# Rayman96/Paddle_ray

Hardware: AMD Instinct MI355X
Metric: tokens/sec GPT-3-1.3B Fleet sharding-3 (higher is better)
Workload: dtype bf16; 1 GPU; model=GPT-3-1.3B, global_batch=16, seq_len=1024, parallelism=sharding3_dp1, micro_batch_per_gpu=16, optimizer=AdamW fp32-master, global-norm clip, zero3_active=False, zero3_params=n/a (world 1)

## Files before the change

paddle_ray_amd/ops/csrc/flash_attn.hip:

```cpp
#include "common.h"
#include "pra_api.h"
#include <stdlib.h>
#include <string.h>
#include <type_traits>
#include <algorithm>
#include <cmath>

namespace pra {
namespace fa {

__device__ __forceinline__ float fexp2(float x) { return __builtin_amdgcn_exp2f(x); }

__device__ __forceinline__ void wait_vmem_all() { __builtin_amdgcn_s_waitcnt(0x0F70); }

typedef float f32x16 __attribute__((ext_vector_type(16)));
typedef uint32_t u32x4 __attribute__((ext_vector_type(4)));
typedef uint32_t u32x2 __attribute__((ext_vector_type(2)));

template <typename T> struct V8;
template <> struct V8<bf16> { typedef __bf16 type __attribute__((ext_vector_type(8))); };
template <> struct V8<f16> { typedef _Float16 type __attribute__((ext_vector_type(8))); };

template <typename T>
__device__ __forceinline__ f32x16 mfma(typename V8<T>::type a, typename V8<T>::type b, f32x16 c);
template <>
__device__ __forceinline__ f32x16 mfma<bf16>(V8<bf16>::type a, V8<bf16>::type b, f32x16 c) {
  return __builtin_amdgcn_mfma_f32_32x32x16_bf16(a, b, c, 0, 0, 0);
}
template <>
__device__ __forceinline__ f32x16 mfma<f16>(V8<f16>::type a, V8<f16>::type b, f32x16 c) {
  return __builtin_amdgcn_mfma_f32_32x32x16_f16(a, b, c, 0, 0, 0);
}

template <typename T> __device__ __forceinline__ uint32_t pack2(float a, float b);
template <> __device__ __forceinline__ uint32_t pack2<bf16>(float a, float b) { return pack_bf2(a, b); }
template <> __device__ __forceinline__ uint32_t pack2<f16>(float a, float b) {
  _Float16 x = (_Float16)a, y = (_Float16)b;
  return (uint32_t)__builtin_bit_cast(uint16_t, x) | ((uint32_t)__builtin_bit_cast(uint16_t, y) << 16);
}
template <typename T> __device__ __forceinline__ float lo16(uint32_t w);
template <typename T> __device__ __forceinline__ float hi16(uint32_t w);
template <> __device__ __forceinline__ float lo16<bf16>(uint32_t w) { return __uint_as_float(w << 16); }
template <> __device__ __forceinline__ float hi16<bf16>(uint32_t w) { return __uint_as_float(w & 0xffff0000u); }
template <> __device__ __forceinline__ float lo16<f16>(uint32_t w) {
  return (float)__builtin_bit_cast(_Float16, (uint16_t)(w & 0xffff));
}
template <> __device__ __forceinline__ float hi16<f16>(uint32_t w) {
  return (float)__builtin_bit_cast(_Float16, (uint16_t)(w >> 16));
}

template <typename T>
__device__ __forceinline__ typename V8<T>::type as_v8(u32x4 u) {
  return __builtin_bit_cast(typename V8<T>::type, u);
}
template <typename T>
__device__ __forceinline__ typename V8<T>::type pack_frag(const f32x16& acc, int base) {
  u32x4 u;
  u[0] = pack2<T>(acc[base + 0], acc[base + 1]);
  u[1] = pack2<T>(acc[base + 2], acc[base + 3]);
  u[2] = pack2<T>(acc[base + 4], acc[base + 5]);
  u[3] = pack2<T>(acc[base + 6], acc[base + 7]);
  return as_v8<T>(u);
}

constexpr int kTile = 64;

struct FaExt {
  const int* cu_q;
  const int* cu_k;
  const void* mask;
  int64_t msb, msh, msq;
  int mask_f32;
  float mask_mul;
  uint32_t thr;
  float inv_keep;
  uint64_t seed, offset;
  uint32_t* dbits;
  int dbits_ld;
  int xf;
  const uint64_t* dseq;
  float* bsum;
  int bsum_nblk;
};

enum : int { XF_DROP = 1, XF_KMASK = 2, XF_FMASK = 4 };

__device__ __forceinline__ uint32_t fa_mix32(uint32_t x) {
  x ^= x >> 16; x *= 0x7feb352dU; x ^= x >> 15; x *= 0x846ca68bU; x ^= x >> 16;
  return x;
}
__device__ __forceinline__ uint32_t fa_key(const FaExt& e, int bh) {
  const uint64_t seed = e.dseq ? e.seed ^ (*e.dseq * 0x9E3779B97F4A7C15ull) : e.seed;
  return fa_mix32((uint32_t)seed ^ (uint32_t)(seed >> 32) * 0x27d4eb2fU ^
                  (uint32_t)e.offset * 0x165667b1U ^ (uint32_t)bh * 0xc2b2ae3dU);
}
__device__ __forceinline__ uint32_t fa_hash2(uint32_t key, int q, int kpair) {
  return fa_mix32(key ^ (uint32_t)q * 0x9e3779b1U ^ (uint32_t)kpair * 0x85ebca77U);
}
__device__ __forceinline__ float fa_keep(const FaExt& e, uint32_t u16) { return u16 >= e.thr ? e.inv_keep : 0.f; }
__device__ __forceinline__ float fa_drop(const FaExt& e, uint32_t key, int q, int kk) {
  const uint32_t hs = fa_hash2(key, q, kk >> 1);
  return fa_keep(e, (kk & 1) ? (hs >> 16) : (hs & 0xffffu));
}
template <typename T>
__device__ __forceinline__ float fa_mask(const FaExt& e, int b, int hh, int q, int kk) {
  const int64_t i = (int64_t)b * e.msb + (int64_t)hh * e.msh + (int64_t)q * e.msq + kk;
  float m;
  if (e.mask_f32) m = static_cast<const float*>(e.mask)[i];
  else m = Cvt<T>::to(static_cast<const T*>(e.mask)[i]);
  return m * e.mask_mul;
}

template <int D>
__device__ __forceinline__ int swz(int row, int ch) {
  return (row >> 3) * (8 * D) + (ch >> 2) * 256 + (row & 7) * 32 + 8 * ((ch & 3) ^ ((row >> 2) & 3));
}
// ... 302 lines not shown
          const uint32_t hs = fa_hash2(dkey, myq, kk >> 1);
          const bool keep = ((i & 1) ? (hs >> 16) : (hs & 0xffffu)) >= ext.thr;
          kbits[mt] |= keep ? (1u << acc_row(i, 0)) : 0u;
          p = keep ? p : 0.f;
        }
        s_acc[mt][i] = p;
      }
    if constexpr ((XF & XF_DROP) != 0) {
      if (ext.dbits) {
#pragma unroll
        for (int mt = 0; mt < 2; ++mt) {
          const uint32_t kb = kbits[mt] << (4 * h);
          const uint32_t w = kb | __shfl_xor(kb, 32, 64);
          if (h == 0 && myq < Sq && mt < nlive)
            ext.dbits[((int64_t)bh * SqM + myq) * ext.dbits_ld + (k0 >> 5) + mt] = w;
        }
      }
    }
    ps += __shfl_xor(ps, 32, 64);
    l_run += ps;
#pragma unroll
    for (int ks = 0; ks < 4; ++ks) {
      if (ks < 2 * nlive) {
        const typename V8<T>::type pf = pack_frag<T>(s_acc[ks >> 1], 8 * (ks & 1));
#pragma unroll
        for (int dt = 0; dt < ND; ++dt)
          acc_o[dt] = mfma<T>(ks < 2 ? vfr[ks & 1][dt] : frag_tr<T, D>(Vs, lo, dt, ks), pf, acc_o[dt]);
      }
    }
    }
    asm volatile("s_waitcnt vmcnt(0)" ::: "memory");
    __syncthreads();
  };
  int nfull = min(ntiles, Sk / kTile);
  if (CAUSAL) nfull = min(nfull, (q0 + off + 1) / kTile);
  if (nfull < 0) nfull = 0;
  auto run = [&](auto xf_c) __attribute__((always_inline)) {
    for (int kt = 0; kt < nfull; ++kt) tile(kt, std::false_type{}, xf_c);
    for (int kt = nfull; kt < ntiles; ++kt) tile(kt, std::true_type{}, xf_c);
  };
  if constexpr (!EXT) {
    run(std::integral_constant<int, 0>{});
  } else {
    switch (ext.xf) {
      case XF_DROP: run(std::integral_constant<int, XF_DROP>{}); break;
      case XF_KMASK: run(std::integral_constant<int, XF_KMASK>{}); break;
      case XF_KMASK | XF_DROP: run(std::integral_constant<int, XF_KMASK | XF_DROP>{}); break;
      case XF_FMASK: run(std::integral_constant<int, XF_FMASK>{}); break;
      case XF_FMASK | XF_DROP: run(std::integral_constant<int, XF_FMASK | XF_DROP>{}); break;
      default: run(std::integral_constant<int, 0>{}); break;
    }
  }

  if (myq < Sq) {
    float inv = l_run > 0.f ? 1.f / l_run : 0.f;
    if constexpr (EXT) {
      if (ext.xf & XF_DROP) inv *= ext.inv_keep;
    }
    T* orow = o + (qrow0 + myq) * ((int64_t)H * D) + (int64_t)hh * D;
#pragma unroll
    for (int dt = 0; dt < ND; ++dt)
#pragma unroll
      for (int g = 0; g < 4; ++g) {
        const int d = 32 * dt + 8 * g + 4 * h;
        uint2 w;
        w.x = pack2<T>(acc_o[dt][4 * g + 0] * inv, acc_o[dt][4 * g + 1] * inv);
        w.y = pack2<T>(acc_o[dt][4 * g + 2] * inv, acc_o[dt][4 * g + 3] * inv);
        *reinterpret_cast<uint2*>(orow + d) = w;
      }
    if (h == 0) {
      const float l2 = l_run > 0.f ? (m_run + log2f(l_run)) : INFINITY;
      lse[(int64_t)bh * SqM + myq] = l2 * 0.6931471805599453f;
    }
  }
}

template <typename T, int D, bool CAUSAL, int NW>
__global__ void __launch_bounds__(NW * 64, 2)
bwd_dq_kernel(const T* __restrict__ q, const T* __restrict__ k, const T* __restrict__ v, const T* __restrict__ dO,
              const T* __restrict__ o, const float* __restrict__ lse, float* __restrict__ delta, T* __restrict__ dq, int H, int Sq,
              int Sk, int64_t qsb, int64_t qss, int64_t qsh, int64_t ksb, int64_t kss, int64_t ksh, int64_t vsb,
              int64_t vss, int64_t vsh, int64_t dqsb, int64_t dqss, int64_t dqsh, float scale, float scale_log2) {
  extern __shared__ __attribute__((aligned(16))) char smem[];
  T* img0 = reinterpret_cast<T*>(smem);
  constexpr int NS = D / 16, ND = D / 32, BM = NW * 32;
  const float LOG2E = 1.4426950408889634f;

  const int nqb = gridDim.y;
  const int qb = CAUSAL ? (nqb - 1 - blockIdx.y) : blockIdx.y;
  const int bh = blockIdx.x, b = bh / H, hh = bh % H;
  const int wave = threadIdx.x >> 6, lane = threadIdx.x & 63, r = lane & 31, h = lane >> 5;
  const int q0 = qb * BM;
  const int myq = q0 + wave * 32 + r;
  const int off = Sk - Sq;
  const bool qvalid = myq < Sq;

  const T* qb_ = q + b * qsb + hh * qsh;
  const T* kb_ = k + b * ksb + hh * ksh;
  const T* vb_ = v + b * vsb + hh * vsh;
  const int64_t HD = (int64_t)H * D;
  const T* dob_ = dO + (int64_t)b * Sq * HD + (int64_t)hh * D;

  typename V8<T>::type qf[NS], df[NS];
  {
    const int qq = qvalid ? myq : 0;
#pragma unroll
    for (int s = 0; s < NS; ++s) {
      qf[s] = frag_global<T>(qb_ + (int64_t)qq * qss, 16 * s + 8 * h, qvalid);
      df[s] = frag_global<T>(dob_ + (int64_t)qq * HD, 16 * s + 8 * h, qvalid);
    }
  }
  const float lse2 = qvalid ? lse[(int64_t)bh * Sq + myq] * LOG2E : INFINITY;
  float dlt;
  if (o) {
    const T* ob_ = o + (int64_t)b * Sq * HD + (int64_t)hh * D;
    const int qq = qvalid ? myq : 0;
    float part = 0.f;
#pragma unroll
    for (int s = 0; s < NS; ++s) {
      const typename V8<T>::type of = frag_global<T>(ob_ + (int64_t)qq * HD, 16 * s + 8 * h, qvalid);
      const u32x4 uo = __builtin_bit_cast(u32x4, of), ud = __builtin_bit_cast(u32x4, df[s]);
#pragma unroll
      for (int j = 0; j < 4; ++j)
// ... 52 lines not shown
#pragma unroll
      for (int g = 0; g <= NG; ++g) {
        if (g < NG) {
#pragma unroll
          for (int j = 0; j < G; ++j) {
            const int f = g * G + j;
            fr[g & 1][j] = f < NS ? frag_rows<T, D>(Ks, lo, mt, f) : frag_rows<T, D>(Vs, lo, mt, f - NS);
          }
        }
        if (g > 0) {
#pragma unroll
          for (int j = 0; j < G; ++j) {
            const int f = (g - 1) * G + j;
            if (f < NS) s_acc[mt] = mfma<T>(fr[(g - 1) & 1][j], qf[f], s_acc[mt]);
            else dp_acc[mt] = mfma<T>(fr[(g - 1) & 1][j], df[f - NS], dp_acc[mt]);
          }
        }
        __builtin_amdgcn_sched_barrier(0);
      }
    }
#pragma unroll
    for (int mt = 0; mt < 2; ++mt)
#pragma unroll
      for (int i = 0; i < 16; ++i) {
        float p = fexp2(fmaf(s_acc[mt][i], scale_log2, -lse2));
        if constexpr (MASK) {
          const int key = k0 + 32 * mt + acc_row(i, h);
          if (mt >= nlive || key >= Sk || (CAUSAL && key > myq + off)) p = 0.f;
        }
        s_acc[mt][i] = p * (dp_acc[mt][i] - dlt);
      }
#pragma unroll
    for (int ks = 0; ks < 4; ++ks) {
      if (ks < 2 * nlive) {
        const typename V8<T>::type sf = pack_frag<T>(s_acc[ks >> 1], 8 * (ks & 1));
#pragma unroll
        for (int dt = 0; dt < ND; ++dt) acc_q[dt] = mfma<T>(frag_tr<T, D>(Ks, lo, dt, ks), sf, acc_q[dt]);
      }
    }
    }
    if (kt + 1 < ntiles) {
      T* nb = img0 + (2 * ((kt + 1) & 1)) * kTile * D;
      kr.store_swz(nb);
      vr.store_swz(nb + kTile * D);
    }
    __syncthreads();
  };
  int nfull = min(ntiles, Sk / kTile);
  if (CAUSAL) nfull = min(nfull, (q0 + off + 1) / kTile);
  if (nfull < 0) nfull = 0;
  for (int kt = 0; kt < nfull; ++kt) tile(kt, std::false_type{});
  for (int kt = nfull; kt < ntiles; ++kt) tile(kt, std::true_type{});

  if (qvalid) {
    T* row = dq + (int64_t)b * dqsb + (int64_t)myq * dqss + (int64_t)hh * dqsh;
#pragma unroll
    for (int dt = 0; dt < ND; ++dt)
#pragma unroll
      for (int g = 0; g < 4; ++g) {
        const int d = 32 * dt + 8 * g + 4 * h;
        uint2 w;
        w.x = pack2<T>(acc_q[dt][4 * g + 0] * scale, acc_q[dt][4 * g + 1] * scale);
        w.y = pack2<T>(acc_q[dt][4 * g + 2] * scale, acc_q[dt][4 * g + 3] * scale);
        *reinterpret_cast<uint2*>(row + d) = w;
      }
  }
}

template <typename T, int D, bool EXT, int NWV = 4>
__host__ __device__ constexpr int kKvOff() {
  return 4 * kTile * D * (int)sizeof(T) + 4 * kTile * 4 + NWV * 32 * 80 + (EXT ? 2 * 256 * 4 : 0);
}
template <typename T, int D, bool EXT, int NWV = 4>
__host__ __device__ constexpr int kDkdvLds() {
  return kKvOff<T, D, EXT, NWV>() + 4 * kTile * D * (int)sizeof(T);
}
__host__ __device__ constexpr int dkdv_waves(bool qs) { return qs ? 8 : 4; }

template <typename T, int D, bool CAUSAL, bool WDS, bool EXT = false, bool QS = false>
__global__ void __launch_bounds__(64 * dkdv_waves(QS), (D == 64 && !QS) ? 2 : 1)
bwd_dkdv_kernel(const T* __restrict__ q, const T* __restrict__ k, const T* __restrict__ v, const T* __restrict__ dO,
                const float* __restrict__ lse, const float* __restrict__ delta, T* __restrict__ dk,
                T* __restrict__ dv, int H, int SqM, int SkM, int64_t qsb, int64_t qss, int64_t qsh, int64_t ksb,
                int64_t kss, int64_t ksh, int64_t vsb, int64_t vss, int64_t vsh, int64_t dksb, int64_t dkss,
                int64_t dksh, int64_t dvsb, int64_t dvss, int64_t dvsh, float scale, float scale_log2,
                T* __restrict__ dsT, int Sqp, int64_t dsbh, FaExt ext = {}) {
  extern __shared__ __attribute__((aligned(16))) char smem[];
  T* img0 = reinterpret_cast<T*>(smem);
  float* Lsb = reinterpret_cast<float*>(img0 + 4 * kTile * D);
  float* Dlb = Lsb + 2 * kTile;
  constexpr int NS = D / 16, ND = D / 32;
  const float LOG2E = 1.4426950408889634f;

  constexpr int NWV = dkdv_waves(QS), NTH = 64 * NWV;
  const int kb = blockIdx.y;
  const int bh = blockIdx.x, b = bh / H, hh = bh % H;
  const int wave = threadIdx.x >> 6, lane = threadIdx.x & 63, r = lane & 31, h = lane >> 5;
  const int kw = QS ? (wave & 3) : wave, qh = QS ? (wave >> 2) : 0;
  const int kblk0 = kb * 128;
  const int mykey = kblk0 + kw * 32 + r;
  int Sq = SqM, Sk = SkM;
  int64_t qrow0 = (int64_t)b * SqM, krow0 = 0;
  if constexpr (EXT) {
    if (ext.cu_q) {
      qrow0 = ext.cu_q[b];
      krow0 = ext.cu_k[b];
      Sq = ext.cu_q[b + 1] - (int)qrow0;
      Sk = ext.cu_k[b + 1] - (int)krow0;
      if (kblk0 >= Sk) return;
    }
  }
  const int off = Sk - Sq;
  const bool kvalid = mykey < Sk;
  const bool vl = EXT && ext.cu_q;

  const T* qb_ = vl ? q + qrow0 * qss + hh * qsh : q + b * qsb + hh * qsh;
  const T* kb_ = vl ? k + krow0 * kss + hh * ksh : k + b * ksb + hh * ksh;
  const T* vb_ = vl ? v + krow0 * vss + hh * vsh : v + b * vsb + hh * vsh;
  const int64_t HD = (int64_t)H * D;
  const T* dob_ = dO + qrow0 * HD + (int64_t)hh * D;

  const T* kvimg = reinterpret_cast<const T*>(smem + kKvOff<T, D, EXT, NWV>());
  const T* Kw = kvimg + (kw >> 1) * kTile * D;
  const T* Vw = kvimg + (2 + (kw >> 1)) * kTile * D;
  f32x16 acc_k[ND], acc_v[ND];
#pragma unroll
  for (int i = 0; i < ND; ++i) { acc_k[i] = f32x16{}; acc_v[i] = f32x16{}; }

  int q_begin = 0;
  if (CAUSAL) q_begin = max(0, kblk0 - off) / kTile * kTile;
  const int ntiles = q_begin < Sq ? (Sq - q_begin + kTile - 1) / kTile : 0;

  const uint32_t lds0 = (uint32_t)(uintptr_t)(__attribute__((address_space(3))) char*)smem;
  SwzDma<D, NTH> qd, dd;
  qd.init(qb_, qss, Sq, wave, lane);
  dd.init(dob_, HD, Sq, wave, lane);
  const bool dbits = EXT && ext.thr && ext.dbits;
  uint32_t* Mb = reinterpret_cast<uint32_t*>(reinterpret_cast<char*>(Dlb + 2 * kTile) + NWV * 32 * 80);
  const uint32_t mb0 = (uint32_t)(uintptr_t)(__attribute__((address_space(3))) char*)Mb;
  const uint32_t lsb0 = (uint32_t)(uintptr_t)(__attribute__((address_space(3))) char*)Lsb;
  const uint32_t dlb0 = (uint32_t)(uintptr_t)(__attribute__((address_space(3))) char*)Dlb;
  const u32x4 lse_rs = raw_desc(lse + (int64_t)bh * SqM, (uint64_t)Sq * 4);
  const u32x4 dl_rs = raw_desc(delta + (int64_t)bh * SqM, (uint64_t)Sq * 4);
  const u32x4 mb_rs = dbits ? raw_desc(ext.dbits + (int64_t)bh * SqM * ext.dbits_ld, (uint64_t)Sq * ext.dbits_ld * 4)
                            : u32x4{0u, 0u, 0u, 0u};
  auto load_tile = [&](int qs0) {
    const int nb = ((qs0 - q_begin) / kTile) & 1;
    const uint32_t img = lds0 + (uint32_t)((2 * nb) * kTile * D * sizeof(T));
    qd.issue(img, (uint32_t)((int64_t)qs0 * qss * 2), wave);
    dd.issue(img + kTile * D * sizeof(T), (uint32_t)((int64_t)qs0 * HD * 2), wave);
    if (wave == 0) dma_dword(lse_rs, (uint32_t)(qs0 + lane) * 4u, lsb0 + nb * kTile * 4);
    if (wave == 1) dma_dword(dl_rs, (uint32_t)(qs0 + lane) * 4u, dlb0 + nb * kTile * 4);
    if (dbits && wave < 4) {
      const int kwd = (kblk0 >> 5) + wave;
      const uint32_t off = kwd < ext.dbits_ld ? (uint32_t)(((int64_t)(qs0 + lane) * ext.dbits_ld + kwd) * 4) : 0x80000000u;
      dma_dword(mb_rs, off, mb0 + (nb * 256 + wave * 64) * 4);
    }
  };
  {
    SwzDma<D, NTH> kd2, vd2;
    kd2.init(kb_, kss, Sk, wave, lane);
    vd2.init(vb_, vss, Sk, wave, lane);
    const uint32_t kv0 = lds0 + (uint32_t)kKvOff<T, D, EXT, NWV>();
#pragma unroll
    for (int j = 0; j < 2; ++j) {
      kd2.issue(kv0 + (uint32_t)(j * kTile * D * sizeof(T)), (uint32_t)((int64_t)(kblk0 + 64 * j) * kss * 2), wave);
      vd2.issue(kv0 + (uint32_t)((2 + j) * kTile * D * sizeof(T)), (uint32_t)((int64_t)(kblk0 + 64 * j) * vss * 2),
// ... 141 lines not shown
            const int i = 4 * g + c;
            const int qq = qs0 + 32 * nt + 8 * g + 4 * h + c;
            float sv = sa[nt][i];
            if constexpr ((XF & XF_FMASK) != 0) {
              if (qq < Sq && kvalid) sv += fa_mask<T>(ext, b, hh, qq, mykey);
            } else if constexpr ((XF & XF_KMASK) != 0) {
              sv += kmv;
            }
            float p = fexp2(fmaf(sv, scale_log2, -la[c]));
            if constexpr (MASK) {
              if (qq >= Sq || (CAUSAL && mykey > qq + off)) p = 0.f;
            }
            if constexpr ((XF & XF_DROP) != 0) {
              const float z = (mwa[c] >> (mykey & 31)) & 1u ? ext.inv_keep : 0.f;
              sa[nt][i] = p * z;
              da[nt][i] = p * (da[nt][i] * z - dl[c]);
              continue;
            }
            sa[nt][i] = p;
            da[nt][i] = p * (da[nt][i] - dl[c]);
          }
        }
#pragma unroll
        for (int ks = 0; ks < 2; ++ks) {
          typename V8<T>::type dtr[ND], qtr[ND];
#pragma unroll
          for (int dt = 0; dt < ND; ++dt) {
            dtr[dt] = frag_tr<T, D>(Ds, lo, dt, 2 * nt + ks);
            qtr[dt] = frag_tr<T, D>(Qs, lo, dt, 2 * nt + ks);
          }
          const typename V8<T>::type pf = pack_frag<T>(sa[nt], 8 * ks);
          const typename V8<T>::type sf = pack_frag<T>(da[nt], 8 * ks);
          if constexpr (WDS) store_ds(sf, ks);
#pragma unroll
          for (int dt = 0; dt < ND; ++dt) {
            acc_v[dt] = mfma<T>(dtr[dt], pf, acc_v[dt]);
            acc_k[dt] = mfma<T>(qtr[dt], sf, acc_k[dt]);
          }
        }
        if constexpr (WDS) flush_ds(qs0 + 32 * nt);
      }
    }
    if constexpr (WDS) wait_vm<QS ? 2 : 4>();
    else wait_vm<0>();
    __builtin_amdgcn_s_waitcnt(0xC07F);
    __builtin_amdgcn_s_barrier();
  };
  int it0 = 0;
  if (CAUSAL) {
    while (it0 < ntiles && kblk0 + 127 > q_begin + it0 * kTile + off) ++it0;
  }
  int it1 = ntiles;
  while (it1 > it0 && q_begin + (it1 - 1) * kTile + kTile > Sq) --it1;
  auto run = [&](auto xf_c) __attribute__((always_inline)) {
    for (int it = 0; it < it0; ++it) tile(it, std::true_type{}, xf_c);
    for (int it = it0; it < it1; ++it) tile(it, std::false_type{}, xf_c);
    for (int it = it1; it < ntiles; ++it) tile(it, std::true_type{}, xf_c);
  };
  if constexpr (!EXT) {
    run(std::integral_constant<int, 0>{});
  } else {
    switch (ext.xf) {
      case XF_DROP: run(std::integral_constant<int, XF_DROP>{}); break;
      case XF_KMASK: run(std::integral_constant<int, XF_KMASK>{}); break;
      case XF_KMASK | XF_DROP: run(std::integral_constant<int, XF_KMASK | XF_DROP>{}); break;
      case XF_FMASK: run(std::integral_constant<int, XF_FMASK>{}); break;
      case XF_FMASK | XF_DROP: run(std::integral_constant<int, XF_FMASK | XF_DROP>{}); break;
      default: run(std::integral_constant<int, 0>{}); break;
    }
  }

  if constexpr (QS) {
    float* xa = reinterpret_cast<float*>(smem);
    __builtin_amdgcn_s_waitcnt(0xC07F);
    __syncthreads();
    if (qh == 1) {
#pragma unroll
      for (int dt = 0; dt < ND; ++dt)
#pragma unroll
        for (int e = 0; e < 16; ++e) {
          xa[((kw * 2 * ND + dt) * 16 + e) * 64 + lane] = acc_k[dt][e];
          xa[((kw * 2 * ND + ND + dt) * 16 + e) * 64 + lane] = acc_v[dt][e];
        }
    }
    __syncthreads();
    if (qh == 0) {
#pragma unroll
      for (int dt = 0; dt < ND; ++dt)
#pragma unroll
        for (int e = 0; e < 16; ++e) {
          acc_k[dt][e] += xa[((kw * 2 * ND + dt) * 16 + e) * 64 + lane];
          acc_v[dt][e] += xa[((kw * 2 * ND + ND + dt) * 16 + e) * 64 + lane];
        }
    }
    __syncthreads();
  }
  constexpr int RP = D + 4;
  T* sk = img0;
  T* sv = img0 + 128 * RP;
  const bool bs = ext.bsum != nullptr;
  if (bs && !QS) {
    __builtin_amdgcn_s_waitcnt(0xC07F);
    __syncthreads();
  }
  const bool writer = !QS || qh == 0;
  T* krow = (vl ? dk + krow0 * dkss : dk + (int64_t)b * dksb) + (int64_t)mykey * dkss + (int64_t)hh * dksh;
  T* vrow = (vl ? dv + krow0 * dvss : dv + (int64_t)b * dvsb) + (int64_t)mykey * dvss + (int64_t)hh * dvsh;
  const int srow = kw * 32 + r;
  if (writer)
#pragma unroll
  for (int dt = 0; dt < ND; ++dt)
#pragma unroll
    for (int g = 0; g < 4; ++g) {
      const int d = 32 * dt + 8 * g + 4 * h;
      uint2 wk, wv;
      wk.x = pack2<T>(acc_k[dt][4 * g + 0] * scale, acc_k[dt][4 * g + 1] * scale);
      wk.y = pack2<T>(acc_k[dt][4 * g + 2] * scale, acc_k[dt][4 * g + 3] * scale);
      wv.x = pack2<T>(acc_v[dt][4 * g + 0], acc_v[dt][4 * g + 1]);
      wv.y = pack2<T>(acc_v[dt][4 * g + 2], acc_v[dt][4 * g + 3]);
      if (kvalid) {
        *reinterpret_cast<uint2*>(krow + d) = wk;
        *reinterpret_cast<uint2*>(vrow + d) = wv;
      }
      if (bs) {
        const uint2 z = make_uint2(0u, 0u);
        *reinterpret_cast<uint2*>(sk + srow * RP + d) = kvalid ? wk : z;
        *reinterpret_cast<uint2*>(sv + srow * RP + d) = kvalid ? wv : z;
      }
    }
  if (bs) {
    __syncthreads();
    const int col = threadIdx.x;
    if (col < 2 * D) {
      const T* src = col < D ? sk + col : sv + (col - D);
      float a = 0.f;
#pragma unroll 8
      for (int i = 0; i < 128; ++i) a += Cvt<T>::to(src[i * RP]);
      const int64_t HD = (int64_t)H * D;
      ext.bsum[((int64_t)b * ext.bsum_nblk + kb) * 3 * HD + (col < D ? 1 : 2) * HD + (int64_t)hh * D + (col % D)] = a;
    }
  }
}

template <typename T, int D, bool CAUSAL, bool EXT = false, int NW = 8, int NBUF = 3>
__global__ void __launch_bounds__(NW * 64, 1)
bwd_dq_ds_kernel(const T* __restrict__ k, const T* __restrict__ dsT, T* __restrict__ dq, int H, int SqM, int SkM,
                 int Sqp, int64_t dsbh, int64_t ksb, int64_t kss, int64_t ksh, int64_t dqsb, int64_t dqss,
                 int64_t dqsh, float scale, FaExt ext = {}) {
  constexpr int NT = NW * 64, BM = NW * 32, ND = D / 32, BUF = kTile * D + kTile * BM;
  static_assert(NBUF >= 2 && NBUF <= 4, "ring depth");
  extern __shared__ __attribute__((aligned(1024))) char smem[];
  T* img0 = reinterpret_cast<T*>(smem);
  const uint32_t lds0 = (uint32_t)(uintptr_t)(__attribute__((address_space(3))) char*)smem;

  const int nqb = gridDim.y;
  const int qb = CAUSAL ? (nqb - 1 - blockIdx.y) : blockIdx.y;
  const int bh = blockIdx.x, b = bh / H, hh = bh % H;
  const int wave = threadIdx.x >> 6, lane = threadIdx.x & 63, r = lane & 31, h = lane >> 5;
  const int q0 = qb * BM;
  const int myq = q0 + wave * 32 + r;
  int Sq = SqM, Sk = SkM;
  int64_t qrow0 = 0, krow0 = 0;
  const bool vl = EXT && ext.cu_q;
  if constexpr (EXT) {
    if (ext.cu_q) {
      qrow0 = ext.cu_q[b];
      krow0 = ext.cu_k[b];
      Sq = ext.cu_q[b + 1] - (int)qrow0;
      Sk = ext.cu_k[b + 1] - (int)krow0;
      if (q0 >= Sq) return;
    }
  }
  const int off = Sk - Sq;

  f32x16 acc_q[ND];
#pragma unroll
  for (int i = 0; i < ND; ++i) acc_q[i] = f32x16{};

  int n_end = Sk;
  if (CAUSAL) n_end = min(Sk, q0 + BM + off);
  const int ntiles = n_end > 0 ? (n_end + kTile - 1) / kTile : 0;

  const LaneOffs<D> lo(lane);
  const LaneOffs<BM> ls(lane);
  SwzDma<D, NT> kd;
  SwzDma<BM, NT> sd;
  kd.init(vl ? k + krow0 * kss + hh * ksh : k + b * ksb + hh * ksh, kss, Sk, wave, lane);
  sd.init(dsT + (int64_t)bh * dsbh + q0, Sqp, Sk, wave, lane);
  auto stage = [&](int kt) {
    const uint32_t img = lds0 + (uint32_t)((kt % NBUF) * BUF * sizeof(T));
    kd.issue(img, (uint32_t)((int64_t)kt * kTile * kss * 2), wave);
    sd.issue(img + kTile * D * sizeof(T), (uint32_t)((int64_t)kt * kTile * Sqp * 2), wave);
  };
  constexpr int PER = SwzDma<D, NT>::PER + SwzDma<BM, NT>::PER;
// ... 5 lines not shown
  else if (staged == NBUF - 1 && NBUF == 3) wait_vm<PER>();
  else if (staged == 2 && NBUF == 4) wait_vm<PER>();
  else asm volatile("s_waitcnt vmcnt(0)" ::: "memory");
  __syncthreads();

  auto tile = [&](int kt, auto mask_c) {
    constexpr bool MASK = decltype(mask_c)::value;
    const int k0 = kt * kTile;
    const T* Ks = img0 + (kt % NBUF) * BUF;
    const T* Ss = Ks + kTile * D;
    const bool ahead = kt + NBUF - 1 < ntiles;
    if (ahead) stage(kt + NBUF - 1);
    int nlive = 2;
    if constexpr (MASK) {
      int kmax = Sk - 1;
      if (CAUSAL) kmax = min(kmax, q0 + wave * 32 + 31 + off);
      nlive = k0 > kmax ? 0 : (k0 + 32 > kmax ? 1 : 2);
      nlive = __builtin_amdgcn_readfirstlane(nlive);
    }
#pragma unroll
    for (int ks = 0; ks < 4; ++ks) {
      if (ks < 2 * nlive) {
        typename V8<T>::type bf = frag_tr<T, BM>(Ss, ls, wave, ks);
        if constexpr (MASK && CAUSAL) {
          u32x4 u = __builtin_bit_cast(u32x4, bf);
          const int kb0 = k0 + 16 * ks + 4 * h - off;
#pragma unroll
          for (int w = 0; w < 4; ++w) {
            const int key_lo = kb0 + 8 * (w >> 1) + 2 * (w & 1);
            const uint32_t mlo = key_lo > myq ? 0u : 0xffffu, mhi = key_lo + 1 > myq ? 0u : 0xffff0000u;
            u[w] &= (mlo | mhi);
          }
          bf = as_v8<T>(u);
        }
        typename V8<T>::type af[ND];
#pragma unroll
        for (int dt = 0; dt < ND; ++dt) af[dt] = frag_tr<T, D>(Ks, lo, dt, ks);
#pragma unroll
        for (int dt = 0; dt < ND; ++dt) acc_q[dt] = mfma<T>(af[dt], bf, acc_q[dt]);
      }
    }
    const int inflight = min(ntiles - 1 - (kt + 1), NBUF - 2);
    if (NBUF == 4 && inflight >= 2) wait_vm<2 * PER>();
    else if (inflight >= 1) wait_vm<PER>();
    else asm volatile("s_waitcnt vmcnt(0)" ::: "memory");
    __syncthreads();
  };
  int nfull = min(ntiles, Sk / kTile);
  if (CAUSAL) nfull = min(nfull, (q0 + off + 1) / kTile);
  if (nfull < 0) nfull = 0;
  for (int kt = 0; kt < nfull; ++kt) tile(kt, std::false_type{});
  for (int kt = nfull; kt < ntiles; ++kt) tile(kt, std::true_type{});

  constexpr int RP = D + 4;
  static_assert(BM * RP <= NBUF * BUF, "dQ stage fits the ring");
  T* sq = img0;
  const bool bs = ext.bsum != nullptr;
  if (bs) {
    __builtin_amdgcn_s_waitcnt(0xC07F);
    __syncthreads();
  }
  const bool qvalid = myq < Sq;
  T* row = (vl ? dq + qrow0 * dqss : dq + (int64_t)b * dqsb) + (int64_t)myq * dqss + (int64_t)hh * dqsh;
#pragma unroll
  for (int dt = 0; dt < ND; ++dt)
#pragma unroll
    for (int g = 0; g < 4; ++g) {
      const int d = 32 * dt + 8 * g + 4 * h;
      uint2 w;
      w.x = pack2<T>(acc_q[dt][4 * g + 0] * scale, acc_q[dt][4 * g + 1] * scale);
      w.y = pack2<T>(acc_q[dt][4 * g + 2] * scale, acc_q[dt][4 * g + 3] * scale);
      if (qvalid) *reinterpret_cast<uint2*>(row + d) = w;
      if (bs) *reinterpret_cast<uint2*>(sq + (wave * 32 + r) * RP + d) = qvalid ? w : make_uint2(0u, 0u);
    }
  if (bs) {
    __syncthreads();
    for (int t = threadIdx.x; t < D * (BM / 128); t += NT) {
      const int half = t / D, col = t % D, blk = (q0 >> 7) + half;
      if (blk >= ext.bsum_nblk) continue;
      const T* src = sq + half * 128 * RP + col;
      float a = 0.f;
#pragma unroll 8
      for (int i = 0; i < 128; ++i) a += Cvt<T>::to(src[i * RP]);
      ext.bsum[((int64_t)b * ext.bsum_nblk + blk) * 3 * (int64_t)H * D + (int64_t)hh * D + col] = a;
    }
  }
}

template <typename T, int D, bool C, int NW>
static void launch_fwd_nw(const void* q, const void* k, const void* v, void* o, float* lse, int B, int H, int Sq,
                          int Sk, const int64_t* st, float scale, hipStream_t s) {
  const size_t lds = 4 * kTile * D * sizeof(T);
  auto kern = fwd_kernel<T, D, C, NW>;
  hipFuncSetAttribute((const void*)kern, hipFuncAttributeMaxDynamicSharedMemorySize, (int)lds);
  dim3 grid(B * H, (Sq + NW * 32 - 1) / (NW * 32));
  hipLaunchKernelGGL(kern, grid, dim3(NW * 64), lds, s, (const T*)q, (const T*)k, (const T*)v, (T*)o, lse, H, Sq, Sk,
                     st[0], st[1], st[2], st[3], st[4], st[5], st[6], st[7], st[8], scale * 1.4426950408889634f,
                     FaExt{});
}

template <typename T, int D, bool C>
static void launch_fwd(const void* q, const void* k, const void* v, void* o, float* lse, int B, int H, int Sq,
                       int Sk, const int64_t* st, float scale, hipStream_t s) {
  if (C) launch_fwd_nw<T, D, C, 4>(q, k, v, o, lse, B, H, Sq, Sk, st, scale, s);
  else launch_fwd_nw<T, D, C, 8>(q, k, v, o, lse, B, H, Sq, Sk, st, scale, s);
}

static int dq_variant() {
  static int v = -1;
  if (v < 0) {
    const char* e = getenv("PRA_FA_DQ_SHAPE");
    v = 0;
    if (e && !strcmp(e, "8x2")) v = 1;
    else if (e && !strcmp(e, "4x3")) v = 2;
    else if (e && !strcmp(e, "4x4")) v = 3;
  }
  return v;
}

template <typename T, int D, bool C, bool EXT, int NW, int NBUF>
static void launch_dq_ds_cfg(const void* k, void* dsT, void* dq, int B, int H, int Sq, int Sk, int Sqp, int64_t dsbh,
                             const int64_t* st, float scale, const FaExt& ext, hipStream_t s) {
  const size_t lds = (size_t)NBUF * (kTile * D + kTile * NW * 32) * sizeof(T);
  auto kern = bwd_dq_ds_kernel<T, D, C, EXT, NW, NBUF>;
  hipFuncSetAttribute((const void*)kern, hipFuncAttributeMaxDynamicSharedMemorySize, (int)lds);
  hipLaunchKernelGGL(kern, dim3(B * H, (Sq + NW * 32 - 1) / (NW * 32)), dim3(NW * 64), lds, s, (const T*)k,
                     (const T*)dsT, (T*)dq, H, Sq, Sk, Sqp, dsbh, st[3], st[4], st[5], st[9], st[10], st[11], scale,
                     ext);
}

template <typename T, int D, bool C, bool EXT>
static void launch_dq_ds(const void* k, void* dsT, void* dq, int B, int H, int Sq, int Sk, int Sqp, int64_t dsbh,
                         const int64_t* st, float scale, const FaExt& ext, hipStream_t s) {
  switch (dq_variant()) {
    case 1: launch_dq_ds_cfg<T, D, C, EXT, 8, 2>(k, dsT, dq, B, H, Sq, Sk, Sqp, dsbh, st, scale, ext, s); break;
    case 2: launch_dq_ds_cfg<T, D, C, EXT, 4, 3>(k, dsT, dq, B, H, Sq, Sk, Sqp, dsbh, st, scale, ext, s); break;
    case 3: launch_dq_ds_cfg<T, D, C, EXT, 4, 4>(k, dsT, dq, B, H, Sq, Sk, Sqp, dsbh, st, scale, ext, s); break;
    default: launch_dq_ds_cfg<T, D, C, EXT, 8, 3>(k, dsT, dq, B, H, Sq, Sk, Sqp, dsbh, st, scale, ext, s); break;
// ... 74 lines not shown
                     st[0], st[1], st[2], st[3], st[4], st[5], st[6], st[7], st[8], scale * 1.4426950408889634f, ext);
}

template <typename T, int D, bool C>
static void launch_bwd_ext(const void* q, const void* k, const void* v, const void* dO, const float* lse,
                           const float* delta, void* dq, void* dk, void* dv, void* dsT, int B, int H, int Sq, int Sk,
                           const int64_t* st, float scale, const FaExt& ext, hipStream_t s) {
  const float sl2 = scale * 1.4426950408889634f;
  const int Sqp = (Sq + 255) / 256 * 256;
  const int64_t dsbh = (int64_t)((Sk + 127) / 128 * 128) * Sqp;
  auto go = [&](auto qs_c) {
    constexpr bool QS = decltype(qs_c)::value;
    const size_t lds = kDkdvLds<T, D, true, dkdv_waves(QS)>();
    auto kern = bwd_dkdv_kernel<T, D, C, true, true, QS>;
    hipFuncSetAttribute((const void*)kern, hipFuncAttributeMaxDynamicSharedMemorySize, (int)lds);
    hipLaunchKernelGGL(kern, dim3(B * H, (Sk + 127) / 128), dim3(64 * dkdv_waves(QS)), lds, s, (const T*)q,
                       (const T*)k, (const T*)v, (const T*)dO, lse, delta, (T*)dk, (T*)dv, H, Sq, Sk, st[0], st[1],
                       st[2], st[3], st[4], st[5], st[6], st[7], st[8], st[12], st[13], st[14], st[15], st[16],
                       st[17], scale, sl2, (T*)dsT, Sqp, dsbh, ext);
  };
  if (D == 128 && dkdv_qs()) go(std::true_type{});
  else go(std::false_type{});
  launch_dq_ds<T, D, C, true>(k, dsT, dq, B, H, Sq, Sk, Sqp, dsbh, st, scale, ext, s);
}

}
}

using namespace pra;

#define PRA_FA_DISPATCH(FN, ...)                                                                  \
  do {                                                                                             \
    if (dt == kBF16) {                                                                             \
      if (D == 128) { if (causal) fa::FN<bf16, 128, true>(__VA_ARGS__); else fa::FN<bf16, 128, false>(__VA_ARGS__); } \
      else { if (causal) fa::FN<bf16, 64, true>(__VA_ARGS__); else fa::FN<bf16, 64, false>(__VA_ARGS__); } \
    } else {                                                                                       \
      if (D == 128) { if (causal) fa::FN<f16, 128, true>(__VA_ARGS__); else fa::FN<f16, 128, false>(__VA_ARGS__); } \
      else { if (causal) fa::FN<f16, 64, true>(__VA_ARGS__); else fa::FN<f16, 64, false>(__VA_ARGS__); } \
    }                                                                                              \
  } while (0)

static fa::FaExt fa_ext(const int* cu_q, const int* cu_k, const void* mask, int64_t msb, int64_t msh, int64_t msq,
                        int mask_f32, float scale, float p_drop, uint64_t seed, uint64_t offset, uint32_t* dbits,
                        int Sk, const uint64_t* dseq) {
  uint32_t thr = (uint32_t)std::min<long long>(65535, std::llround((double)p_drop * 65536.0));
  int xf = 0;
  if (thr > 0) xf |= fa::XF_DROP;
  if (mask) xf |= (msq == 0 && Sk <= 4096) ? fa::XF_KMASK : fa::XF_FMASK;
  return fa::FaExt{cu_q, cu_k, mask, msb, msh, msq, mask_f32, 1.f / scale, thr,
                   thr > 0 ? (float)(65536.0 / (65536.0 - thr)) : 1.f, seed, offset, dbits, (Sk + 31) / 32, xf,
                   dseq};
}

extern "C" {
int pra_flash_fwd(const void* q, const void* k, const void* v, void* o, float* lse, int B, int H, int Sq, int Sk,
                  int D, const int64_t* strides, float scale, int causal, int dt, hipStream_t s) {
  if (!(D == 64 || D == 128) || !(dt == kBF16 || dt == kF16)) return -1;
  if (B * H == 0 || Sq == 0) return 0;
  PRA_FA_DISPATCH(launch_fwd, q, k, v, o, lse, B, H, Sq, Sk, strides, scale, s);
  return 0;
}
int pra_flash_fwd_ext(const void* q, const void* k, const void* v, void* o, float* lse, int B, int H, int Sq, int Sk,
                      int D, const int64_t* strides, float scale, int causal, int dt, const int* cu_q,
                      const int* cu_k, const void* mask, int64_t msb, int64_t msh, int64_t msq, int mask_f32,
                      float p_drop, uint64_t seed, uint64_t offset, uint32_t* dbits, const uint64_t* dseq,
                      hipStream_t s) {
  if (!(D == 64 || D == 128) || !(dt == kBF16 || dt == kF16)) return -1;
  if (!(p_drop >= 0.f && p_drop < 1.f) || (!cu_q) != (!cu_k)) return -1;
  if (B * H == 0 || Sq == 0) return 0;
  const fa::FaExt e = fa_ext(cu_q, cu_k, mask, msb, msh, msq, mask_f32, scale, p_drop, seed, offset, dbits, Sk, dseq);
  PRA_FA_DISPATCH(launch_fwd_ext, q, k, v, o, lse, B, H, Sq, Sk, strides, scale, e, s);
  return 0;
}
int pra_flash_bwd_ext(const void* q, const void* k, const void* v, const void* dO, const float* lse,
                      const float* delta, void* dq, void* dk, void* dv, void* dsT, int B, int H, int Sq, int Sk, int D,
                      const int64_t* strides, float scale, int causal, int dt, const int* cu_q, const int* cu_k,
                      const void* mask, int64_t msb, int64_t msh, int64_t msq, int mask_f32, float p_drop,
                      uint64_t seed, uint64_t offset, uint32_t* dbits, const uint64_t* dseq, float* bsum,
                      hipStream_t s) {
  if (!(D == 64 || D == 128) || !(dt == kBF16 || dt == kF16) || !dsT) return -1;
  if (!(p_drop >= 0.f && p_drop < 1.f) || (!cu_q) != (!cu_k)) return -1;
  if (bsum && (cu_q || Sq != Sk)) return -4;
  if (B * H == 0 || Sq == 0) return 0;
  fa::FaExt e = fa_ext(cu_q, cu_k, mask, msb, msh, msq, mask_f32, scale, p_drop, seed, offset, dbits, Sk, dseq);
  e.bsum = bsum;
  e.bsum_nblk = (Sk + 127) / 128;
  if ((e.xf & fa::XF_DROP) && !dbits) return -3;
  PRA_FA_DISPATCH(launch_bwd_ext, q, k, v, dO, lse, delta, dq, dk, dv, dsT, B, H, Sq, Sk, strides, scale, e, s);
  return 0;
}
int pra_flash_bwd(const void* q, const void* k, const void* v, const void* dO, const void* o, const float* lse,
                  float* delta, void* dq, void* dk, void* dv, void* dsT, int B, int H, int Sq, int Sk, int D,
                  const int64_t* strides, float scale, int causal, int dt, float* bsum, hipStream_t s) {
  if (!(D == 64 || D == 128) || !(dt == kBF16 || dt == kF16)) return -1;
  if (dsT && o) return -2;
  if (bsum && (!dsT || Sq != Sk)) return -4;
  if (B * H == 0 || Sq == 0) return 0;
  PRA_FA_DISPATCH(launch_bwd, q, k, v, dO, o, lse, delta, dq, dk, dv, dsT, B, H, Sq, Sk, strides, scale, bsum, s);
  return 0;
}
}
```

Before: 131,000 tokens/s.

## Widen flash-attention epilogue stores with permlane32 swaps and split column-sum reductions

Rewrites the epilogues of the forward, dQ and dK/dV kernels so lane halves exchange packed pairs via permlane32_swap. Each lane then issues 16-byte stores instead of 8-byte ones, and host-side alignment checks reject misaligned outputs. The QS reduction in dK/dV now exchanges float4 chunks so both wave halves each finalise one of K or V, dropping a barrier and splitting the writer role. The bias column sums are spread across all threads with a partial-sum pass, and the LDS row pitch grows to D+8. It also adds optional timestamp instrumentation, which is compiled out by default. Risks include extra LDS usage, an extra barrier in the bsum path, and new -5 failures for misaligned tensors.

```diff
diff --git a/paddle_ray_amd/ops/csrc/flash_attn.hip b/paddle_ray_amd/ops/csrc/flash_attn.hip
--- a/paddle_ray_amd/ops/csrc/flash_attn.hip
+++ b/paddle_ray_amd/ops/csrc/flash_attn.hip
@@ -62,6 +62,41 @@
   u[3] = pack2<T>(acc[base + 6], acc[base + 7]);
   return as_v8<T>(u);
 }
+
+__device__ __forceinline__ u32x4 widen_pair(uint2 a, uint2 b) {
+  const auto rx = __builtin_amdgcn_permlane32_swap(a.x, b.x, false, false);
+  const auto ry = __builtin_amdgcn_permlane32_swap(a.y, b.y, false, false);
+  return u32x4{rx[0], ry[0], rx[1], ry[1]};
+}
+template <typename T>
+__device__ __forceinline__ u32x4 out_piece(const f32x16& acc, int gp, float mul) {
+  uint2 a, b;
+  a.x = pack2<T>(acc[8 * gp + 0] * mul, acc[8 * gp + 1] * mul);
+  a.y = pack2<T>(acc[8 * gp + 2] * mul, acc[8 * gp + 3] * mul);
+  b.x = pack2<T>(acc[8 * gp + 4] * mul, acc[8 * gp + 5] * mul);
+  b.y = pack2<T>(acc[8 * gp + 6] * mul, acc[8 * gp + 7] * mul);
+  return widen_pair(a, b);
+}
+
+#ifndef PRA_FA_STAMPS
+#define PRA_FA_STAMPS 0
+#endif
+#if PRA_FA_STAMPS
+__device__ unsigned long long g_fa_stamps[2][8][8];
+#define FA_STAMP(i)                                                                               \
+  do {                                                                                            \
+    if (blockIdx.x == 0 && (blockIdx.y == 0 || blockIdx.y == gridDim.y - 1) && (threadIdx.x & 63) == 0) \
+      g_fa_stamps[blockIdx.y != 0][threadIdx.x >> 6][i] = __builtin_amdgcn_s_memtime();          \
+  } while (0)
+#define FA_STAMP_VAL(i, v)                                                                        \
+  do {                                                                                            \
+    if (blockIdx.x == 0 && (blockIdx.y == 0 || blockIdx.y == gridDim.y - 1) && (threadIdx.x & 63) == 0) \
+      g_fa_stamps[blockIdx.y != 0][threadIdx.x >> 6][i] = (unsigned long long)(v);               \
+  } while (0)
+#else
+#define FA_STAMP(i) do {} while (0)
+#define FA_STAMP_VAL(i, v) do {} while (0)
+#endif
 
 constexpr int kTile = 64;
 
@@ -470,23 +505,21 @@
     }
   }
 
-  if (myq < Sq) {
+  {
+    const bool qvalid = myq < Sq;
     float inv = l_run > 0.f ? 1.f / l_run : 0.f;
     if constexpr (EXT) {
       if (ext.xf & XF_DROP) inv *= ext.inv_keep;
     }
-    T* orow = o + (qrow0 + myq) * ((int64_t)H * D) + (int64_t)hh * D;
+    T* orow = o + (qrow0 + myq) * ((int64_t)H * D) + (int64_t)hh * D + 8 * h;
 #pragma unroll
     for (int dt = 0; dt < ND; ++dt)
 #pragma unroll
-      for (int g = 0; g < 4; ++g) {
-        const int d = 32 * dt + 8 * g + 4 * h;
-        uint2 w;
-        w.x = pack2<T>(acc_o[dt][4 * g + 0] * inv, acc_o[dt][4 * g + 1] * inv);
-        w.y = pack2<T>(acc_o[dt][4 * g + 2] * inv, acc_o[dt][4 * g + 3] * inv);
-        *reinterpret_cast<uint2*>(orow + d) = w;
-      }
-    if (h == 0) {
+      for (int gp = 0; gp < 2; ++gp) {
+        const u32x4 w = out_piece<T>(acc_o[dt], gp, inv);
+        if (qvalid) *reinterpret_cast<u32x4*>(orow + 32 * dt + 16 * gp) = w;
+      }
+    if (qvalid && h == 0) {
       const float l2 = l_run > 0.f ? (m_run + log2f(l_run)) : INFINITY;
       lse[(int64_t)bh * SqM + myq] = l2 * 0.6931471805599453f;
     }
@@ -645,17 +678,14 @@
   for (int kt = 0; kt < nfull; ++kt) tile(kt, std::false_type{});
   for (int kt = nfull; kt < ntiles; ++kt) tile(kt, std::true_type{});
 
-  if (qvalid) {
-    T* row = dq + (int64_t)b * dqsb + (int64_t)myq * dqss + (int64_t)hh * dqsh;
+  {
+    T* row = dq + (int64_t)b * dqsb + (int64_t)myq * dqss + (int64_t)hh * dqsh + 8 * h;
 #pragma unroll
     for (int dt = 0; dt < ND; ++dt)
 #pragma unroll
-      for (int g = 0; g < 4; ++g) {
-        const int d = 32 * dt + 8 * g + 4 * h;
-        uint2 w;
-        w.x = pack2<T>(acc_q[dt][4 * g + 0] * scale, acc_q[dt][4 * g + 1] * scale);
-        w.y = pack2<T>(acc_q[dt][4 * g + 2] * scale, acc_q[dt][4 * g + 3] * scale);
-        *reinterpret_cast<uint2*>(row + d) = w;
+      for (int gp = 0; gp < 2; ++gp) {
+        const u32x4 w = out_piece<T>(acc_q[dt], gp, scale);
+        if (qvalid) *reinterpret_cast<u32x4*>(row + 32 * dt + 16 * gp) = w;
       }
   }
 }
@@ -706,6 +736,7 @@
   const int off = Sk - Sq;
   const bool kvalid = mykey < Sk;
   const bool vl = EXT && ext.cu_q;
+  FA_STAMP(0);
 
   const T* qb_ = vl ? q + qrow0 * qss + hh * qsh : q + b * qsb + hh * qsh;
   const T* kb_ = vl ? k + krow0 * kss + hh * ksh : k + b * ksb + hh * ksh;
@@ -953,6 +984,8 @@
   }
   int it1 = ntiles;
   while (it1 > it0 && q_begin + (it1 - 1) * kTile + kTile > Sq) --it1;
+  FA_STAMP(1);
+  FA_STAMP_VAL(7, ntiles);
   auto run = [&](auto xf_c) __attribute__((always_inline)) {
     for (int it = 0; it < it0; ++it) tile(it, std::true_type{}, xf_c);
     for (int it = it0; it < it1; ++it) tile(it, std::false_type{}, xf_c);
@@ -971,76 +1004,88 @@
     }
   }
 
+  FA_STAMP(2);
   if constexpr (QS) {
-    float* xa = reinterpret_cast<float*>(smem);
+    float4* xa = reinterpret_cast<float4*>(smem);
+    float4* mine = xa + wave * (4 * ND) * 64 + lane;
+    const float4* theirs = xa + (wave ^ 4) * (4 * ND) * 64 + lane;
     __builtin_amdgcn_s_waitcnt(0xC07F);
     __syncthreads();
-    if (qh == 1) {
+    auto park = [&](const f32x16* acc) __attribute__((always_inline)) {
 #pragma unroll
       for (int dt = 0; dt < ND; ++dt)
 #pragma unroll
-        for (int e = 0; e < 16; ++e) {
-          xa[((kw * 2 * ND + dt) * 16 + e) * 64 + lane] = acc_k[dt][e];
-          xa[((kw * 2 * ND + ND + dt) * 16 + e) * 64 + lane] = acc_v[dt][e];
-        }
-    }
+        for (int g = 0; g < 4; ++g)
+          mine[(dt * 4 + g) * 64] = make_float4(acc[dt][4 * g], acc[dt][4 * g + 1], acc[dt][4 * g + 2], acc[dt][4 * g + 3]);
+    };
+    auto fetch = [&](f32x16* acc) __attribute__((always_inline)) {
+#pragma unroll
+      for (int dt = 0; dt < ND; ++dt)
+#pragma unroll
+        for (int g = 0; g < 4; ++g) {
+          const float4 x = theirs[(dt * 4 + g) * 64];
+          acc[dt][4 * g] += x.x;
+          acc[dt][4 * g + 1] += x.y;
+          acc[dt][4 * g + 2] += x.z;
+          acc[dt][4 * g + 3] += x.w;
+        }
+    };
+    if (qh == 0) park(acc_v);
+    else park(acc_k);
     __syncthreads();
-    if (qh == 0) {
-#pragma unroll
-      for (int dt = 0; dt < ND; ++dt)
-#pragma unroll
-        for (int e = 0; e < 16; ++e) {
-          acc_k[dt][e] += xa[((kw * 2 * ND + dt) * 16 + e) * 64 + lane];
-          acc_v[dt][e] += xa[((kw * 2 * ND + ND + dt) * 16 + e) * 64 + lane];
-        }
-    }
-    __syncthreads();
-  }
-  constexpr int RP = D + 4;
+    if (qh == 0) fetch(acc_k);
+    else fetch(acc_v);
+  }
+  FA_STAMP(3);
+  constexpr int RP = D + 8;
   T* sk = img0;
   T* sv = img0 + 128 * RP;
   const bool bs = ext.bsum != nullptr;
-  if (bs && !QS) {
+  if (bs) {
     __builtin_amdgcn_s_waitcnt(0xC07F);
     __syncthreads();
   }
-  const bool writer = !QS || qh == 0;
-  T* krow = (vl ? dk + krow0 * dkss : dk + (int64_t)b * dksb) + (int64_t)mykey * dkss + (int64_t)hh * dksh;
-  T* vrow = (vl ? dv + krow0 * dvss : dv + (int64_t)b * dvsb) + (int64_t)mykey * dvss + (int64_t)hh * dvsh;
   const int srow = kw * 32 + r;
-  if (writer)
-#pragma unroll
-  for (int dt = 0; dt < ND; ++dt)
-#pragma unroll
-    for (int g = 0; g < 4; ++g) {
-      const int d = 32 * dt + 8 * g + 4 * h;
-      uint2 wk, wv;
-      wk.x = pack2<T>(acc_k[dt][4 * g + 0] * scale, acc_k[dt][4 * g + 1] * scale);
-      wk.y = pack2<T>(acc_k[dt][4 * g + 2] * scale, acc_k[dt][4 * g + 3] * scale);
-      wv.x = pack2<T>(acc_v[dt][4 * g + 0], acc_v[dt][4 * g + 1]);
-      wv.y = pack2<T>(acc_v[dt][4 * g + 2], acc_v[dt][4 * g + 3]);
-      if (kvalid) {
-        *reinterpret_cast<uint2*>(krow + d) = wk;
-        *reinterpret_cast<uint2*>(vrow + d) = wv;
-      }
-      if (bs) {
-        const uint2 z = make_uint2(0u, 0u);
-        *reinterpret_cast<uint2*>(sk + srow * RP + d) = kvalid ? wk : z;
-        *reinterpret_cast<uint2*>(sv + srow * RP + d) = kvalid ? wv : z;
-      }
-    }
+  auto emit = [&](const f32x16* acc, float mul, T* base, int64_t rs, int64_t hs, int64_t bsd, T* st) __attribute__((always_inline)) {
+    T* row = (vl ? base + krow0 * rs : base + (int64_t)b * bsd) + (int64_t)mykey * rs + (int64_t)hh * hs + 8 * h;
+#pragma unroll
+    for (int dt = 0; dt < ND; ++dt)
+#pragma unroll
+      for (int gp = 0; gp < 2; ++gp) {
+        const u32x4 w = out_piece<T>(acc[dt], gp, mul);
+        if (kvalid) *reinterpret_cast<u32x4*>(row + 32 * dt + 16 * gp) = w;
+        if (bs) *reinterpret_cast<u32x4*>(st + srow * RP + 32 * dt + 16 * gp + 8 * h) = kvalid ? w : u32x4{0u, 0u, 0u, 0u};
+      }
+  };
+  if (!QS || qh == 0) emit(acc_k, scale, dk, dkss, dksh, dksb, sk);
+  if (!QS || qh == 1) emit(acc_v, 1.f, dv, dvss, dvsh, dvsb, sv);
+  FA_STAMP(4);
   if (bs) {
     __syncthreads();
-    const int col = threadIdx.x;
-    if (col < 2 * D) {
-      const T* src = col < D ? sk + col : sv + (col - D);
-      float a = 0.f;
+    constexpr int NP = NTH / (2 * D);
+    static_assert(NP >= 1 && NP * 2 * D == NTH && 128 % NP == 0, "column-sum split");
+    const int col = threadIdx.x % (2 * D), part = threadIdx.x / (2 * D);
+    const T* src = (col < D ? sk + col : sv + (col - D)) + part * (128 / NP) * RP;
+    float a = 0.f;
 #pragma unroll 8
-      for (int i = 0; i < 128; ++i) a += Cvt<T>::to(src[i * RP]);
+    for (int i = 0; i < 128 / NP; ++i) a += Cvt<T>::to(src[i * RP]);
+    if constexpr (NP > 1) {
+      float* ps = reinterpret_cast<float*>(sv + 128 * RP);
+      if (part > 0) ps[(part - 1) * 2 * D + col] = a;
+      __syncthreads();
+#pragma unroll
+      for (int p = 1; p < NP; ++p) a += ps[(p - 1) * 2 * D + col];
+    }
+    if (part == 0) {
       const int64_t HD = (int64_t)H * D;
       ext.bsum[((int64_t)b * ext.bsum_nblk + kb) * 3 * HD + (col < D ? 1 : 2) * HD + (int64_t)hh * D + (col % D)] = a;
     }
   }
+  FA_STAMP(5);
+#if PRA_FA_STAMPS
+  wait_vm<0>();
+#endif
+  FA_STAMP(6);
 }
 
 template <typename T, int D, bool CAUSAL, bool EXT = false, int NW = 8, int NBUF = 3>
@@ -1152,8 +1197,10 @@
   for (int kt = 0; kt < nfull; ++kt) tile(kt, std::false_type{});
   for (int kt = nfull; kt < ntiles; ++kt) tile(kt, std::true_type{});
 
-  constexpr int RP = D + 4;
-  static_assert(BM * RP <= NBUF * BUF, "dQ stage fits the ring");
+  constexpr int RP = D + 8;
+  constexpr int NCOL = D * (BM / 128), NP = NT / NCOL;
+  static_assert(NP >= 1 && NP * NCOL == NT && 128 % NP == 0, "column-sum split");
+  static_assert((BM * RP * (int)sizeof(T) + (NP - 1) * NCOL * 4) <= NBUF * BUF * (int)sizeof(T), "dQ stage fits the ring");
   T* sq = img0;
   const bool bs = ext.bsum != nullptr;
   if (bs) {
@@ -1161,29 +1208,32 @@
     __syncthreads();
   }
   const bool qvalid = myq < Sq;
-  T* row = (vl ? dq + qrow0 * dqss : dq + (int64_t)b * dqsb) + (int64_t)myq * dqss + (int64_t)hh * dqsh;
+  T* row = (vl ? dq + qrow0 * dqss : dq + (int64_t)b * dqsb) + (int64_t)myq * dqss + (int64_t)hh * dqsh + 8 * h;
 #pragma unroll
   for (int dt = 0; dt < ND; ++dt)
 #pragma unroll
-    for (int g = 0; g < 4; ++g) {
-      const int d = 32 * dt + 8 * g + 4 * h;
-      uint2 w;
-      w.x = pack2<T>(acc_q[dt][4 * g + 0] * scale, acc_q[dt][4 * g + 1] * scale);
-      w.y = pack2<T>(acc_q[dt][4 * g + 2] * scale, acc_q[dt][4 * g + 3] * scale);
-      if (qvalid) *reinterpret_cast<uint2*>(row + d) = w;
-      if (bs) *reinterpret_cast<uint2*>(sq + (wave * 32 + r) * RP + d) = qvalid ? w : make_uint2(0u, 0u);
+    for (int gp = 0; gp < 2; ++gp) {
+      const u32x4 w = out_piece<T>(acc_q[dt], gp, scale);
+      if (qvalid) *reinterpret_cast<u32x4*>(row + 32 * dt + 16 * gp) = w;
+      if (bs) *reinterpret_cast<u32x4*>(sq + (wave * 32 + r) * RP + 32 * dt + 16 * gp + 8 * h) = qvalid ? w : u32x4{0u, 0u, 0u, 0u};
     }
   if (bs) {
     __syncthreads();
-    for (int t = threadIdx.x; t < D * (BM / 128); t += NT) {
-      const int half = t / D, col = t % D, blk = (q0 >> 7) + half;
-      if (blk >= ext.bsum_nblk) continue;
-      const T* src = sq + half * 128 * RP + col;
-      float a = 0.f;
+    const int t = threadIdx.x % NCOL, part = threadIdx.x / NCOL;
+    const int half = t / D, col = t % D, blk = (q0 >> 7) + half;
+    const T* src = sq + (half * 128 + part * (128 / NP)) * RP + col;
+    float a = 0.f;
 #pragma unroll 8
-      for (int i = 0; i < 128; ++i) a += Cvt<T>::to(src[i * RP]);
+    for (int i = 0; i < 128 / NP; ++i) a += Cvt<T>::to(src[i * RP]);
+    if constexpr (NP > 1) {
+      float* ps = reinterpret_cast<float*>(sq + BM * RP);
+      if (part > 0) ps[(part - 1) * NCOL + t] = a;
+      __syncthreads();
+#pragma unroll
+      for (int p = 1; p < NP; ++p) a += ps[(p - 1) * NCOL + t];
+    }
+    if (part == 0 && blk < ext.bsum_nblk)
       ext.bsum[((int64_t)b * ext.bsum_nblk + blk) * 3 * (int64_t)H * D + (int64_t)hh * D + col] = a;
-    }
   }
 }
 
@@ -1364,11 +1414,23 @@
                    dseq};
 }
 
+static bool fa_out_ok(const void* p, const int64_t* st3 = nullptr) {
+  if ((uintptr_t)p & 15) return false;
+  return !st3 || ((st3[0] | st3[1] | st3[2]) & 7) == 0;
+}
+
 extern "C" {
+#if PRA_FA_STAMPS
+int pra_flash_stamps_read(unsigned long long* out, hipStream_t s) {
+  if (hipStreamSynchronize(s) != hipSuccess) return -1;
+  return hipMemcpyFromSymbol(out, HIP_SYMBOL(fa::g_fa_stamps), sizeof(fa::g_fa_stamps)) == hipSuccess ? 0 : -1;
+}
+#endif
 int pra_flash_fwd(const void* q, const void* k, const void* v, void* o, float* lse, int B, int H, int Sq, int Sk,
                   int D, const int64_t* strides, float scale, int causal, int dt, hipStream_t s) {
   if (!(D == 64 || D == 128) || !(dt == kBF16 || dt == kF16)) return -1;
   if (B * H == 0 || Sq == 0) return 0;
+  if (!fa_out_ok(o)) return -5;
   PRA_FA_DISPATCH(launch_fwd, q, k, v, o, lse, B, H, Sq, Sk, strides, scale, s);
   return 0;
 }
@@ -1380,6 +1442,7 @@
   if (!(D == 64 || D == 128) || !(dt == kBF16 || dt == kF16)) return -1;
   if (!(p_drop >= 0.f && p_drop < 1.f) || (!cu_q) != (!cu_k)) return -1;
   if (B * H == 0 || Sq == 0) return 0;
+  if (!fa_out_ok(o)) return -5;
   const fa::FaExt e = fa_ext(cu_q, cu_k, mask, msb, msh, msq, mask_f32, scale, p_drop, seed, offset, dbits, Sk, dseq);
   PRA_FA_DISPATCH(launch_fwd_ext, q, k, v, o, lse, B, H, Sq, Sk, strides, scale, e, s);
   return 0;
@@ -1394,6 +1457,7 @@
   if (!(p_drop >= 0.f && p_drop < 1.f) || (!cu_q) != (!cu_k)) return -1;
   if (bsum && (cu_q || Sq != Sk)) return -4;
   if (B * H == 0 || Sq == 0) return 0;
+  if (!fa_out_ok(dq, strides + 9) || !fa_out_ok(dk, strides + 12) || !fa_out_ok(dv, strides + 15)) return -5;
   fa::FaExt e = fa_ext(cu_q, cu_k, mask, msb, msh, msq, mask_f32, scale, p_drop, seed, offset, dbits, Sk, dseq);
   e.bsum = bsum;
   e.bsum_nblk = (Sk + 127) / 128;
@@ -1408,6 +1472,7 @@
   if (dsT && o) return -2;
   if (bsum && (!dsT || Sq != Sk)) return -4;
   if (B * H == 0 || Sq == 0) return 0;
+  if (!fa_out_ok(dq, strides + 9) || !fa_out_ok(dk, strides + 12) || !fa_out_ok(dv, strides + 15)) return -5;
   PRA_FA_DISPATCH(launch_bwd, q, k, v, dO, o, lse, delta, dq, dk, dv, dsT, B, H, Sq, Sk, strides, scale, bsum, s);
   return 0;
 }
```

Result: no change. 132,000 tokens/s (median of 6 runs) (+0.7%).
